# g8a9/multi-modal-emotion

Hardware: AMD Instinct MI355X
Metric: utterances/sec fwd+bwd (+clip_grad_norm_+AdamW inside the timed step), TAV (BERT+Wav2Vec2+VideoMAE) b=32, 1/2/4/8 MI355X (higher is better)
Workload: dtype bf16; 1 GPU; tav_nn.py TAV preset B (bert 12 L + wav2vec2 12 L / 768 + videomae 12 L / 768 on 16 frames + fusion 12 L), global batch 32 = 32 per GPU x 1, text 128 tok, audio 80000 samples, video 16x3x224x224 (104 fusion / 1464 encoder tokens), 547.0 GFLOP forward per utterance; global_batch=32, per_gpu_batch=32, parallelism=dp1, weights=random init (seeded), no checkpoints offline, launch=hipGraph replay

## Files before the change

### include/tavhip.h

```cpp
#ifndef TAVHIP_H
#define TAVHIP_H
#include <stdint.h>

#ifdef __cplusplus
extern "C" {
#endif

enum { TAV_F32 = 0, TAV_BF16 = 1, TAV_FP8 = 2  };
enum {
    TAV_ERR_NULL = -1,
    TAV_ERR_SHAPE = -2,
    TAV_ERR_DTYPE = -3,
    TAV_ERR_ALIGN = -4,
    TAV_ERR_NO_RCCL = -5
};

int tav_version(void);
const char* tav_error_string(int code);

typedef struct tav_gemm_nt_args {
    const void* A; const void* B; void* C;
    void* C_pre;
    const float* bias;
    const void* gelu_in;
// ... 120 lines not shown
int tav_embed_add_fwd(const float* x, const int64_t* ids, const float* table, float* out, int64_t rows, int64_t W, int64_t ntable,
                      void* stream);
int tav_embed_add_bwd(const float* dy, const int64_t* ids, float* dtable, float* partials, int64_t rows, int64_t W, int64_t ntable,
                      int32_t accumulate, void* stream);
int tav_embed_add_bwd_parts(int64_t rows);

typedef struct tav_text_embed_args {
    const int64_t* ids;
    const float* word; const float* pos; const float* type;
    const float* gamma; const float* beta;
    float* pre;
    int64_t* pos_ids;
    float* y_f32; void* y_lp; int32_t lp_dtype;
    float* mean; float* rstd;
    int64_t B, S, W, vocab, max_pos;
    int32_t pad_id;
    float eps;
} tav_text_embed_args;
int tav_text_embed_fwd(const tav_text_embed_args* args, void* stream);
int tav_scatter_add_rows(const float* d, const int64_t* idx, float* dtable, int64_t rows, int64_t W, int64_t ntable, void* stream);

int tav_patchify(const float* video, const int32_t* keep_idx, void* patches, int32_t dtype, int64_t B, int64_t F, int64_t H, int64_t W,
                 int64_t nkeep, void* stream);
int tav_mask_to_index(const uint8_t* mask, int32_t keep_value, int32_t* keep_idx, int32_t* counts, int64_t B, int64_t n, int64_t nkeep,
                      void* stream);
enum { TAV_RAGGED_OVER_TRUE = 1, TAV_RAGGED_OVER_KEEP = 2 };
int tav_ragged_lens(const uint8_t* mask, int32_t* true_cnt, int32_t* vid_lens, int32_t* av_lens, int32_t* status, int64_t B, int64_t ntok,
                    int64_t cap_true, int64_t cap_keep, int64_t base, void* stream);
int tav_gather_rows(const float* table, const int32_t* idx, float* out, int64_t rows, int64_t W, int64_t ntable, void* stream);

int tav_mean_pool_fwd(const float* x, float* y, int64_t B, int64_t S, int64_t W, void* stream);
int tav_mean_pool_bwd(const float* dy, float* dx, void* dx_lp, int32_t lp_dtype, int64_t B, int64_t S, int64_t W, void* stream);
int tav_mean_pool_fwd_len(const float* x, float* y, const int32_t* seq_lens, int64_t B, int64_t S, int64_t W, void* stream);
int tav_mean_pool_bwd_len(const float* dy, float* dx, void* dx_lp, int32_t lp_dtype, const int32_t* seq_lens, int64_t B, int64_t S, int64_t W,
                          void* stream);

int tav_head_fwd(const float* x, const float* W, const float* b, float* y, int64_t B, int64_t K, int64_t N, void* stream);
int tav_head_bwd(const float* x, const float* W, const float* dy, float* dx, float* dW, float* db, int64_t B, int64_t K, int64_t N,
                 int32_t accumulate, void* stream);
int tav_tanh_fwd(const float* x, float* y, int64_t n, void* stream);
int tav_tanh_bwd(const float* y, const float* dy, float* dx, int64_t n, void* stream);

int tav_cross_entropy(const float* logits, const int64_t* target, const float* class_weight , float* loss, float* dlogits,
                      int64_t B, int64_t C, float grad_scale, void* stream);

int tav_dropout_fwd(const float* x, float* y, uint8_t* mask, int64_t n, float p, uint64_t seed, uint64_t offset, void* stream);
int tav_dropout_fwd_dev(const float* x, float* y, uint8_t* mask, int64_t n, float p, const uint64_t* seed_state, uint64_t offset, void* stream);
int tav_dropout_bwd(const float* dy, const uint8_t* mask, float* dx, int64_t n, float p, void* stream);

#define TAV_SPECAUG_TAG_TIME 0x5350010000000000ull
#define TAV_SPECAUG_TAG_FEATURE 0x5350030000000000ull
int tav_specaug_draw(const uint8_t* valid, uint8_t* mask, int32_t* nspans, int64_t B, int64_t L, float prob, int64_t length, int64_t min_masks,
                     uint64_t seed, uint64_t tag, void* stream);
int tav_specaug_draw_dev(const uint8_t* valid, uint8_t* mask, int32_t* nspans, int64_t B, int64_t L, float prob, int64_t length,
                         int64_t min_masks, const uint64_t* seed_state, uint64_t tag, void* stream);
int tav_specaug_fwd(const float* x, const uint8_t* tmask, const uint8_t* fmask, const float* embed, float* y, int64_t B, int64_t T, int64_t H,
                    void* stream);
int64_t tav_specaug_bwd_ws_bytes(int64_t rows, int64_t H);
int tav_specaug_bwd(const float* dy, const uint8_t* tmask, const uint8_t* fmask, float* dx, float* dembed, void* workspace,
                    int64_t workspace_bytes, int64_t B, int64_t T, int64_t H, void* stream);

int tav_conv0_fwd(const float* wave, const float* w, const float* bias, void* y, int32_t y_dtype, int64_t B, int64_t T_in, int64_t T_out,
                  int64_t C, int64_t K, int64_t stride, void* stream);
int tav_conv0_bwd_w(const float* wave, const void* dy, int32_t dy_dtype, float* dw, float* dbias, float* partials, int64_t B, int64_t T_in,
                    int64_t T_out, int64_t C, int64_t K, int64_t stride, int32_t accumulate, void* stream);
int tav_conv0_bwd_partials(int64_t B, int64_t T_out, int64_t C, int64_t K);
int tav_gn_workspace_floats(int64_t B, int64_t C);
int tav_gn_gelu_fwd(const void* x, void* y, int32_t dtype, const float* gamma, const float* beta, float* stats, float* workspace, int64_t B,
                    int64_t T, int64_t C, float eps, void* stream);
int tav_gn_gelu_bwd(const void* x, const void* dy, void* dx, int32_t dtype, const float* gamma, const float* beta, const float* stats,
                    float* workspace, float* dgamma, float* dbeta, int64_t B, int64_t T, int64_t C, int32_t accumulate, void* stream);
int tav_gelu_fwd(const void* x, void* y, int32_t dtype, int64_t n, void* stream);
int tav_gelu_bwd(const void* x, const void* dy, void* dx, int32_t dtype, int64_t n, void* stream);
int tav_col2im_1d(const void* dcol, void* dx, const void* pre_act, int32_t dtype, int64_t B, int64_t T_in, int64_t T_out, int64_t C,
                  int64_t K, int64_t stride, void* stream);
int tav_group_pad(const void* x, int32_t x_dtype, void* xg, int32_t xg_dtype, int64_t B, int64_t T, int64_t H, int64_t G, int64_t pad_l,
                  int64_t pad_r, void* stream);
int tav_weight_norm_partials(int64_t H, int64_t Cg);
int tav_weight_norm_fwd(const float* v, const float* g, float* norms, float* partials, void* w, void* w_flip, int32_t dtype, int64_t H,
                        int64_t Cg, int64_t K, void* stream);
int tav_weight_norm_bwd(const float* v, const float* g, const float* norms, const float* dw_gemm, float* workspace, float* dv, float* dg,
                        int64_t H, int64_t Cg, int64_t K, int32_t accumulate, void* stream);

int tav_sumsq_partials(int32_t ntensors);
int tav_sumsq_multi(const float* const* ptrs, const int64_t* sizes, int32_t ntensors, float* partials, float* out_sumsq, void* stream);
int tav_clip_coef(const float* sumsq, float max_norm, float* coef_out, float* norm_out, void* stream);
int tav_adamw_multi(float* const* params, const float* const* grads, float* const* exp_avg, float* const* exp_avg_sq, const int64_t* sizes,
                    int32_t ntensors, const float* clip_coef , const float* lr, float beta1, float beta2, float eps, float weight_decay,
                    int32_t* step, float* bias_corr, void* stream);
int tav_optim_chunk_elems(void);
int tav_sumsq_chunked(const float* const* ptrs, const int64_t* sizes, const int32_t* chunk_prefix, int32_t ntensors, int32_t nchunks,
                      float* partials, float* out_sumsq, void* stream);
int tav_sum_partials(const float* partials, int64_t n, float* out, void* stream);
int tav_adamw_chunked(float* const* params, const float* const* grads, float* const* exp_avg, float* const* exp_avg_sq, const int64_t* sizes,
                      const int32_t* chunk_prefix, int32_t ntensors, int32_t nchunks, const float* clip_coef, const float* lr, float beta1,
                      float beta2, float eps, float weight_decay, int32_t* step, float* bias_corr, void* stream);

int tav_comm_rccl_version(int32_t* version);
int tav_comm_unique_id(void* out128);
int tav_comm_init_rank(void** comm, int32_t nranks, const void* unique_id128, int32_t rank);
int tav_comm_destroy(void* comm);
int tav_allreduce_bucket(void* buf, int64_t nbytes, int32_t dtype, void* comm, void* stream);

#ifdef __cplusplus
}
#endif
#endif
```

### multi-modal-emotion_amd/_lib.py

```python
import ctypes as C
import os

import torch

_HERE = os.path.dirname(os.path.abspath(__file__))
LIB_PATH = os.environ.get("TAV_LIB") or os.path.join(_HERE, "libtavhip.so")

TAV_F32, TAV_BF16, TAV_FP8 = 0, 1, 2
ABI_VERSION = 7

i32, i64, f32, vp = C.c_int32, C.c_int64, C.c_float, C.c_void_p


class GemmNTArgs(C.Structure):
    _fields_ = [("A", vp), ("B", vp), ("C", vp), ("C_pre", vp), ("bias", vp), ("gelu_in", vp), ("resid", vp),
                ("M", i64), ("N", i64), ("K", i64),
                ("lda", i64), ("ldb", i64), ("ldc", i64), ("ld_pre", i64), ("ld_gelu_in", i64), ("ld_resid", i64),
                ("nzb", i32), ("nzg", i32),
                ("a_zb", i64), ("a_zg", i64), ("b_zb", i64), ("b_zg", i64), ("c_zb", i64), ("c_zg", i64), ("bias_zg", i64),
                ("in_dtype", i32), ("out_dtype", i32), ("act", i32), ("accumulate", i32), ("alpha", f32),
                ("a_dequant", vp), ("b_dequant", vp), ("gelu_zb", i64), ("tile_m_hint", i32)]


class GemmTNArgs(C.Structure):
    _fields_ = [("A", vp), ("B", vp), ("slabs", vp), ("out", vp), ("dbias", vp), ("bias_partials", vp),
                ("N1", i64), ("N2", i64), ("lda", i64), ("ldb", i64), ("rows_per_batch", i64), ("nbatch", i64),
                ("a_zb", i64), ("b_zb", i64), ("chunk_rows", i32), ("nsplit", i32), ("perm_inner", i32), ("perm_outer", i32),
                ("dtype", i32), ("accumulate", i32), ("scale", f32)]


class GemmTNProblem(C.Structure):
    _fields_ = [("A", vp), ("B", vp), ("out", vp), ("dbias", vp), ("N1", i64), ("N2", i64), ("lda", i64), ("ldb", i64)]


class AttnArgs(C.Structure):
    _fields_ = [("q", vp), ("k", vp), ("v", vp), ("o", vp), ("key_mask", vp), ("lse", vp), ("corr", vp), ("o_soft", vp),
                ("dout", vp), ("dq", vp), ("dk", vp), ("dv", vp), ("delta", vp),
                ("B", i64), ("S", i64), ("nheads", i64),
                ("ld_q", i64), ("ld_k", i64), ("ld_v", i64), ("ld_o", i64), ("ld_do", i64), ("ld_dq", i64), ("ld_dk", i64), ("ld_dv", i64),
                ("dtype", i32), ("mask_mode", i32), ("scale", f32), ("q_prescaled", i32)]


class LnArgs(C.Structure):
    _fields_ = [("x", vp), ("x_dtype", i32), ("gamma", vp), ("beta", vp), ("y_f32", vp), ("y_lp", vp), ("lp_dtype", i32),
                ("mean", vp), ("rstd", vp),
                ("dy", vp), ("dy_dtype", i32), ("dx_add", vp), ("dx_f32", vp), ("dx_lp", vp),
                ("dgamma", vp), ("dbeta", vp), ("partials", vp), ("accumulate_params", i32),
                ("rows", i64), ("W", i64), ("ld_x", i64), ("ld_y", i64), ("ld_dy", i64), ("ld_dx", i64), ("eps", f32), ("act", i32),
                ("defer_param_reduce", i32)]


class LnReduceItem(C.Structure):
    _fields_ = [("partials", vp), ("dgamma", vp), ("dbeta", vp), ("nblocks", i32), ("W", i32), ("accumulate", i32), ("pad_", i32)]


LN_REDUCE_MAX = 64


class TextEmbedArgs(C.Structure):
    _fields_ = [("ids", vp), ("word", vp), ("pos", vp), ("type", vp), ("gamma", vp), ("beta", vp), ("pre", vp), ("pos_ids", vp),
                ("y_f32", vp), ("y_lp", vp), ("lp_dtype", i32), ("mean", vp), ("rstd", vp),
                ("B", i64), ("S", i64), ("W", i64), ("vocab", i64), ("max_pos", i64), ("pad_id", i32), ("eps", f32)]


_SIGS = {
    "tav_version": (C.c_int, []),
    "tav_error_string": (C.c_char_p, [C.c_int]),
    "tav_gemm_nt": (C.c_int, [C.POINTER(GemmNTArgs), vp]),
    "tav_gemm_nt_schedule": (C.c_int, [C.POINTER(GemmNTArgs), C.POINTER(i32), C.POINTER(i32), C.POINTER(i32)]),
    "tav_gemm_tn_splits": (C.c_int, [i64, i64, i64, i64, C.POINTER(i32), C.POINTER(i32)]),
    "tav_gemm_tn": (C.c_int, [C.POINTER(GemmTNArgs), vp]),
    "tav_gemm_tn_grouped": (C.c_int, [C.POINTER(GemmTNProblem), i32, i64, i32, vp]),
    "tav_gemm_tn_grouped_ws_bytes": (C.c_int64, [C.POINTER(GemmTNProblem), i32, i64, i32, i32]),
    "tav_gemm_tn_grouped_ws": (C.c_int, [C.POINTER(GemmTNProblem), i32, i64, i32, vp, i64, i32, vp]),
    "tav_colsum": (C.c_int, [vp, i32, i64, i64, i64, vp, i32, vp, i32, vp]),
    "tav_fp8_amax_partials": (C.c_int, [i64, i64]),
    "tav_fp8_amax": (C.c_int, [vp, i32, i64, i64, i64, vp, vp, vp]),
    "tav_fp8_quantize": (C.c_int, [vp, i32, i64, i64, i64, vp, vp, i64, vp, i64, i64, vp]),
    "tav_fp8_quantize_delayed": (C.c_int, [vp, i32, i64, i64, i64, vp, vp, i64, vp, i64, i64, vp]),
    "tav_fp8_roll_states": (C.c_int, [vp, i64, vp]),
    "tav_splitk_reduce": (C.c_int, [vp, vp, i32, i64, i32, vp]),
    "tav_comm_rccl_version": (C.c_int, [C.POINTER(i32)]),
    "tav_comm_unique_id": (C.c_int, [vp]),
    "tav_comm_init_rank": (C.c_int, [C.POINTER(vp), i32, vp, i32]),
    "tav_comm_destroy": (C.c_int, [vp]),
    "tav_allreduce_bucket": (C.c_int, [vp, i64, i32, vp, vp]),
    "tav_attn_fwd": (C.c_int, [C.POINTER(AttnArgs), vp]),
    "tav_attn_bwd": (C.c_int, [C.POINTER(AttnArgs), vp]),
    "tav_attn_fwd_len": (C.c_int, [C.POINTER(AttnArgs), vp, vp]),
    "tav_attn_bwd_len": (C.c_int, [C.POINTER(AttnArgs), vp, vp]),
    "tav_attn_probs": (C.c_int, [C.POINTER(AttnArgs), vp, vp, i64, vp]),
    "tav_head_scale": (C.c_int, [vp, vp, vp, i32, vp, i64, f32, i64, i64, i64, i64, i64, i64, vp]),
    "tav_ln_fwd": (C.c_int, [C.POINTER(LnArgs), vp]),
    "tav_ln_bwd": (C.c_int, [C.POINTER(LnArgs), vp]),
    "tav_ln_bwd_partials": (C.c_int, [i64]),
    "tav_ln_param_reduce_multi": (C.c_int, [C.POINTER(LnReduceItem), i32, vp]),
    "tav_cast_weight": (C.c_int, [vp, i64, i64, vp, i64, vp, i64, i32, vp]),
    "tav_cast_weights_multi": (C.c_int, [vp, i32, i32, vp]),
    "tav_cast_conv_weight": (C.c_int, [vp, i64, i64, i64, vp, vp, vp, i64, i32, vp]),
    "tav_zero_pad_rows": (C.c_int, [vp, i32, i64, i64, i64, i64, vp]),
    "tav_cast2d": (C.c_int, [vp, i32, i64, vp, i32, i64, i64, i64, vp]),
    "tav_transpose2d": (C.c_int, [vp, vp, i32, i64, i64, i64, vp]),
    "tav_add_f32": (C.c_int, [vp, vp, vp, vp, i32, i64, vp]),
    "tav_fill_f32": (C.c_int, [vp, f32, i64, vp]),
    "tav_embed_add_fwd": (C.c_int, [vp, vp, vp, vp, i64, i64, i64, vp]),
    "tav_embed_add_bwd": (C.c_int, [vp, vp, vp, vp, i64, i64, i64, i32, vp]),
    "tav_embed_add_bwd_parts": (C.c_int, [i64]),
    "tav_text_embed_fwd": (C.c_int, [C.POINTER(TextEmbedArgs), vp]),
    "tav_scatter_add_rows": (C.c_int, [vp, vp, vp, i64, i64, i64, vp]),
    "tav_gather_rows": (C.c_int, [vp, vp, vp, i64, i64, i64, vp]),
    "tav_patchify": (C.c_int, [vp, vp, vp, i32, i64, i64, i64, i64, i64, vp]),
    "tav_mask_to_index": (C.c_int, [vp, i32, vp, vp, i64, i64, i64, vp]),
    "tav_ragged_lens": (C.c_int, [vp, vp, vp, vp, vp, i64, i64, i64, i64, i64, vp]),
    "tav_mean_pool_fwd": (C.c_int, [vp, vp, i64, i64, i64, vp]),
    "tav_mean_pool_bwd": (C.c_int, [vp, vp, vp, i32, i64, i64, i64, vp]),
    "tav_mean_pool_fwd_len": (C.c_int, [vp, vp, vp, i64, i64, i64, vp]),
    "tav_mean_pool_bwd_len": (C.c_int, [vp, vp, vp, i32, vp, i64, i64, i64, vp]),
    "tav_head_fwd": (C.c_int, [vp, vp, vp, vp, i64, i64, i64, vp]),
    "tav_head_bwd": (C.c_int, [vp, vp, vp, vp, vp, vp, i64, i64, i64, i32, vp]),
    "tav_tanh_fwd": (C.c_int, [vp, vp, i64, vp]),
    "tav_tanh_bwd": (C.c_int, [vp, vp, vp, i64, vp]),
    "tav_cross_entropy": (C.c_int, [vp, vp, vp, vp, vp, i64, i64, f32, vp]),
    "tav_dropout_fwd": (C.c_int, [vp, vp, vp, i64, f32, C.c_uint64, C.c_uint64, vp]),
    "tav_dropout_fwd_dev": (C.c_int, [vp, vp, vp, i64, f32, vp, C.c_uint64, vp]),
    "tav_dropout_bwd": (C.c_int, [vp, vp, vp, i64, f32, vp]),
    "tav_specaug_draw": (C.c_int, [vp, vp, vp, i64, i64, f32, i64, i64, C.c_uint64, C.c_uint64, vp]),
    "tav_specaug_draw_dev": (C.c_int, [vp, vp, vp, i64, i64, f32, i64, i64, vp, C.c_uint64, vp]),
    "tav_specaug_fwd": (C.c_int, [vp, vp, vp, vp, vp, i64, i64, i64, vp]),
    "tav_specaug_bwd_ws_bytes": (C.c_int64, [i64, i64]),
    "tav_specaug_bwd": (C.c_int, [vp, vp, vp, vp, vp, vp, i64, i64, i64, i64, vp]),
    "tav_conv0_fwd": (C.c_int, [vp, vp, vp, vp, i32, i64, i64, i64, i64, i64, i64, vp]),
    "tav_conv0_bwd_w": (C.c_int, [vp, vp, i32, vp, vp, vp, i64, i64, i64, i64, i64, i64, i32, vp]),
    "tav_conv0_bwd_partials": (C.c_int, [i64, i64, i64, i64]),
    "tav_gn_workspace_floats": (C.c_int, [i64, i64]),
    "tav_gn_gelu_fwd": (C.c_int, [vp, vp, i32, vp, vp, vp, vp, i64, i64, i64, f32, vp]),
    "tav_gn_gelu_bwd": (C.c_int, [vp, vp, vp, i32, vp, vp, vp, vp, vp, vp, i64, i64, i64, i32, vp]),
    "tav_gelu_fwd": (C.c_int, [vp, vp, i32, i64, vp]),
    "tav_gelu_bwd": (C.c_int, [vp, vp, vp, i32, i64, vp]),
    "tav_col2im_1d": (C.c_int, [vp, vp, vp, i32, i64, i64, i64, i64, i64, i64, vp]),
    "tav_group_pad": (C.c_int, [vp, i32, vp, i32, i64, i64, i64, i64, i64, i64, vp]),
    "tav_weight_norm_partials": (C.c_int, [i64, i64]),
    "tav_weight_norm_fwd": (C.c_int, [vp, vp, vp, vp, vp, vp, i32, i64, i64, i64, vp]),
    "tav_weight_norm_bwd": (C.c_int, [vp, vp, vp, vp, vp, vp, vp, i64, i64, i64, i32, vp]),
    "tav_sumsq_partials": (C.c_int, [i32]),
    "tav_sumsq_multi": (C.c_int, [vp, vp, i32, vp, vp, vp]),
    "tav_clip_coef": (C.c_int, [vp, f32, vp, vp, vp]),
    "tav_adamw_multi": (C.c_int, [vp, vp, vp, vp, vp, i32, vp, vp, f32, f32, f32, f32, vp, vp, vp]),
    "tav_optim_chunk_elems": (C.c_int, []),
    "tav_sumsq_chunked": (C.c_int, [vp, vp, vp, i32, i32, vp, vp, vp]),
    "tav_sum_partials": (C.c_int, [vp, i64, vp, vp]),
    "tav_adamw_chunked": (C.c_int, [vp, vp, vp, vp, vp, vp, i32, i32, vp, vp, f32, f32, f32, f32, vp, vp, vp]),
}

_lib = None


def lib():
# ... 44 lines not shown
```

### multi-modal-emotion_amd/engine.py

```python
import os
import weakref

import torch

from . import ops

_EPOCH = [0]


def bump_weight_epoch():
    _EPOCH[0] += 1


class Policy:
    def __init__(self, name="bf16"):
        name = {"bfloat16": "bf16", "float32": "fp32", "f32": "fp32", "float8": "fp8", "e4m3": "fp8"}.get(name, name)
        if name not in ("bf16", "fp32", "fp8", "fp8-all", "fp8-wgrad8"):
            raise ValueError(f"unknown precision policy {name!r}")
        self.name = name
        self.lp = torch.float32 if name == "fp32" else torch.bfloat16
        self.f32 = name == "fp32"
        self.fp8 = name.startswith("fp8")
        self.fp8_stacks = () if not self.fp8 else (("video", "text", "audio", "fusion") if name == "fp8-all" else ("video",))
        self.fp8_wgrad8 = name in ("fp8-wgrad8", "fp8-all")
# ... 592 lines not shown
        ctx.ectx, ctx.geom, ctx.has_b = ectx, (B, T_in, Ci, Co, k, stride, T_out), b is not None
        ctx.chained = u_in is not None
        ctx.set_materialize_grads(False)
        ctx.save_for_backward(x, w, pre, u_in)
        return y, pre

    @staticmethod
    def backward(ctx, g, g_pre):
        x, w, pre, u_in = ctx.saved_tensors
        B, T_in, Ci, Co, k, stride, T_out = ctx.geom
        du = g_pre
        if g is not None:
            d2 = ops.gelu_bwd(pre, _c(g)) if pre is not None else _c(g)
            du = d2 if du is None else _c(du) + d2
        if du is None:
            return None, None, None, None, None, None, None
        _, w_t, w_ph = ctx.ectx.cache.conv(w, stride)
        P = CONV_PAD
        TP = T_out + 2 * P
        du_pad = _CONV_PADDED.pop(du.data_ptr(), None) if g is None else None
        if du_pad is not None and (tuple(du.shape) != (B, T_out, Co) or tuple(du.stride()) != (TP * Co, Co, 1) or tuple(du_pad.shape) != (B, TP, Co)):
            du_pad = None
        want_dx = ctx.needs_input_grad[1] if ctx.chained else ctx.needs_input_grad[0]
        phase = (CONV_PHASE_DGRAD[0] and w_ph is not None and want_dx and (k + stride - 1) // stride - 1 <= P
                 and (T_in - 1) // stride + 1 <= T_out + P)
        if du_pad is None:
            du = _c(du)
            if phase and du.numel() <= (1 << 23):
                du_pad = ops.zero_pad_rows(torch.empty(B, TP, Co, dtype=du.dtype, device=du.device), B, T_out, Co, P)
                du_pad[:, P:P + T_out].copy_(du)
            else:
                phase = False
        du_v = du_pad[:, P:P + T_out] if du_pad is not None else du
        za = TP * Co if du_pad is not None else T_out * Co
        dw = db = dx = dui = None
        if ctx.needs_input_grad[2]:
            dw = ops.gemm_tn(du_v, x, N1=Co, N2=k * Ci, lda=Co, ldb=stride * Ci, rows_per_batch=T_out, nbatch=B, a_zb=za, b_zb=T_in * Ci,
                             perm_inner=Ci, perm_outer=k, out_shape=(Co, Ci, k))
        if ctx.has_b and ctx.needs_input_grad[3]:
            db = ops.colsum(du_pad.view(B * TP, Co) if du_pad is not None else du.view(B * T_out, Co))
        if want_dx and phase:
            if ctx.chained:
                out = ops.zero_pad_rows(torch.empty(B, T_in + 2 * P, Ci, dtype=du_v.dtype, device=du_v.device), B, T_in, Ci, P)
                zc, obase = (T_in + 2 * P) * Ci, P * Ci
            else:
                out = torch.empty(B, T_in, Ci, dtype=du_v.dtype, device=du_v.device)
                zc, obase = T_in * Ci, 0
            oflat, aflat, uflat = out.view(-1), du_pad.view(-1), (u_in.reshape(-1) if ctx.chained else None)
            off = 0
            for r in range(stride):
                Q = (k - r + stride - 1) // stride
                Mr = (T_in - r + stride - 1) // stride
                ops.gemm_nt(aflat[(P - (Q - 1)) * Co:], w_ph[off:off + Ci * Q * Co], out=oflat[obase + r * Ci:], M=Mr, N=Ci, K=Q * Co, lda=Co, ldb=Q * Co,
                            ldc=stride * Ci, nzb=B, a_zb=TP * Co, c_zb=zc, gelu_in=uflat[r * Ci:] if ctx.chained else None,
                            ld_gelu=stride * Ci, gelu_zb=T_in * Ci)
                off += Ci * Q * Co
            if ctx.chained:
                dui = out[:, P:P + T_in]
                _CONV_PADDED[dui.data_ptr()] = out
            else:
                dx = out
        elif want_dx:
            dcol = ops.gemm_nt(_c(du_v).view(B * T_out, Co), w_t, out_shape=(B * T_out, k * Ci))
            d = ops.col2im_1d(dcol, B, T_in, T_out, Ci, k, stride, pre_act=u_in if ctx.chained else None)
            if ctx.chained:
                dui = d
            else:
                dx = d
        return dx, dui, dw, db, None, None, None


class PosConvFn(torch.autograd.Function):

    @staticmethod
    def forward(ctx, x, v, g, bias, B, T, G, ectx):
        pol = ectx.pol
        x = _c(x)
        H = x.shape[1]
        Cg, K = H // G, v.shape[2]
        w, _, norms = ectx.cache.posconv(v, g)
        pad = K // 2
        xg = ops.group_pad(x, B, T, H, G, pad, pad, pol.lp)
        TP = T + 2 * pad
        y, pre = ops.gemm_nt(xg, w, bias=bias, act=1, resid=x, want_pre=True, out_dtype=torch.float32, M=T, N=Cg, K=K * Cg, lda=Cg, ldb=K * Cg,
                             ldc=H, nzb=B, nzg=G, a_zb=G * TP * Cg, a_zg=TP * Cg, b_zg=Cg * K * Cg, c_zb=T * H, c_zg=Cg, bias_zg=Cg,
                             out_shape=(B * T, H))
        ctx.ectx, ctx.geom = ectx, (B, T, H, G, Cg, K)
        ctx.save_for_backward(xg, pre, v, g, norms)
        return y

    @staticmethod
    def backward(ctx, gout):
        xg, pre, v, g, norms = ctx.saved_tensors
        pol = ctx.ectx.pol
        B, T, H, G, Cg, K = ctx.geom
        gout = _c(gout)
        _, wf, _ = ctx.ectx.cache.posconv(v, g)
        du = ops.gelu_bwd(pre, gout)
        pad = K // 2
        dug = ops.group_pad(du, B, T, H, G, pad - 1, pad, pol.lp)
        TPd, TP = T + 2 * pad - 1, T + 2 * pad
        dx = ops.gemm_nt(dug, wf, resid=gout, out_dtype=torch.float32, M=T, N=Cg, K=K * Cg, lda=Cg, ldb=K * Cg, ldc=H, nzb=B, nzg=G,
                         a_zb=G * TPd * Cg, a_zg=TPd * Cg, b_zg=Cg * K * Cg, c_zb=T * H, c_zg=Cg, out_shape=(B * T, H))
        du_lp = _to_lp(pol, du)
        dw = torch.empty(G, Cg, K * Cg, dtype=torch.float32, device=du.device)
        for gi in range(G):
            ops.gemm_tn(du_lp[:, gi * Cg:], xg[:, gi], out=dw[gi], N1=Cg, N2=K * Cg, lda=H, ldb=Cg, rows_per_batch=T, nbatch=B, a_zb=T * H,
                        b_zb=G * TP * Cg)
        dv, dg = ops.weight_norm_bwd(v, g, norms, dw)
        dbias = ops.colsum(du)
        return dx, dv, dg.view_as(g), dbias, None, None, None, None


class ConcatSeqFn(torch.autograd.Function):

    @staticmethod
    def forward(ctx, B, *parts):
        W = parts[0].shape[-1]
        lens = [p.numel() // (B * W) for p in parts]
        Sf = sum(lens)
        out = torch.empty(B, Sf, W, dtype=torch.float32, device=parts[0].device)
        flat = out.view(B, Sf * W)
        off = 0
        for p, L in zip(parts, lens):
            ops.cast2d(_c(p).view(B, L * W), torch.float32, out=flat[:, off * W:(off + L) * W])
            off += L
        ctx.lens, ctx.W, ctx.B = lens, W, B
        return out

    @staticmethod
    def backward(ctx, g):
        B, W = ctx.B, ctx.W
        flat = _c(g).view(B, -1)
        outs, off = [], 0
        for L in ctx.lens:
            outs.append(ops.cast2d(flat[:, off * W:(off + L) * W], torch.float32).view(B * L, W))
            off += L
        return (None, *outs)


class TailFn(torch.autograd.Function):

    @staticmethod
    def forward(ctx, av_seq, t_pooled, aud_seq, vid_seq, B, S_av, S_aud, S_vid, p_drop, seed, rand_w, rand_b, bert_w, bert_b, aud_w, aud_b,
                vid_w, vid_b, lin_w, lin_b, av_lens=None, vid_lens=None):
        W = 768
        pooled = [ops.mean_pool_fwd(_c(av_seq), B, S_av, seq_lens=av_lens), _c(t_pooled), ops.mean_pool_fwd(_c(aud_seq), B, S_aud),
                  ops.mean_pool_fwd(_c(vid_seq), B, S_vid, seq_lens=vid_lens)]
        norms = [(rand_w, rand_b), (bert_w, bert_b), (aud_w, aud_b), (vid_w, vid_b)]
        cat = torch.empty(B, 4 * W, dtype=torch.float32, device=av_seq.device)
        stats = []
        for j, (x, (w, b)) in enumerate(zip(pooled, norms)):
            y32, _, mean, rstd = ops.ln_fwd(x, w.detach(), b.detach(), 1e-5, want_f32=True)
            ops.cast2d(y32, torch.float32, out=cat[:, j * W:(j + 1) * W])
            stats += [mean, rstd]
        mask = None
        feat = cat
        if p_drop > 0.0:
            feat, mask = ops.dropout_fwd(cat, p_drop, seed, 0)
        logits = ops.head_fwd(feat, lin_w.detach(), lin_b.detach())
        ctx.geom = (B, S_av, S_aud, S_vid, p_drop)
        ctx.lens = (av_lens, vid_lens)
        ctx.save_for_backward(feat, mask, lin_w, *pooled, *stats, rand_w, rand_b, bert_w, bert_b, aud_w, aud_b, vid_w, vid_b)
        return logits

    @staticmethod
    def backward(ctx, g):
        B, S_av, S_aud, S_vid, p_drop = ctx.geom
        sv = ctx.saved_tensors
        feat, mask, lin_w = sv[:3]
        pooled, stats, nw = sv[3:7], sv[7:15], sv[15:23]
        W = 768
        dfeat, dW, db = ops.head_bwd(feat, lin_w, _c(g))
        if mask is not None:
            dfeat = ops.dropout_bwd(dfeat, mask, p_drop)
        dpool, dparams = [], []
        for j in range(4):
            dy = ops.cast2d(dfeat[:, j * W:(j + 1) * W], torch.float32)
            dx, _, dg, dbt = ops.ln_bwd(dy, pooled[j], nw[2 * j], nw[2 * j + 1], stats[2 * j], stats[2 * j + 1], want_f32=True)
            dpool.append(dx)
            dparams += [dg, dbt]
        av_lens, vid_lens = ctx.lens
        d_av, _ = ops.mean_pool_bwd(dpool[0], B, S_av, seq_lens=av_lens)
        d_aud, _ = ops.mean_pool_bwd(dpool[2], B, S_aud)
        d_vid, _ = ops.mean_pool_bwd(dpool[3], B, S_vid, seq_lens=vid_lens)
        return (d_av, dpool[1], d_aud, d_vid, None, None, None, None, None, None, *dparams, dW, db, None, None)


class HeadFn(torch.autograd.Function):

    @staticmethod
# ... 154 lines not shown
```

### multi-modal-emotion_amd/ops.py

```python
import ctypes as C
import os

import torch

from . import _lib as L
from ._lib import check, dt, lib, ptr, stream

_ws = {}


def workspace(name, nfloats, device):
    key = (name, torch.cuda.current_stream().cuda_stream, str(device))
    t = _ws.get(key)
    if t is None or t.numel() < nfloats:
        t = torch.empty(max(int(nfloats), 1), dtype=torch.float32, device=device)
        _ws[key] = t
    return t


def clear_workspaces():
    _ws.clear()


_prof = None
# ... 657 lines not shown
        check(lib().tav_specaug_draw_dev(ptr(valid), ptr(mask), ptr(nspans), B, L, prob, length, min_masks, ptr(seed), tag, stream()), "specaug_draw_dev")
    else:
        check(lib().tav_specaug_draw(ptr(valid), ptr(mask), ptr(nspans), B, L, prob, length, min_masks, seed, tag, stream()), "specaug_draw")
    return (mask, nspans) if want_nspans else mask


def specaug_fwd(x, tmask, fmask, embed, B, T):
    H = x.shape[-1]
    tmask, fmask = _mask_bytes(tmask, (B, T), "specaug_fwd"), _mask_bytes(fmask, (B, H), "specaug_fwd")
    y = torch.empty_like(x)
    check(lib().tav_specaug_fwd(ptr(x), ptr(tmask), ptr(fmask), ptr(embed), ptr(y), B, T, H, stream()), "specaug_fwd")
    return y


def specaug_bwd(dy, tmask, fmask, B, T, want_dembed=True):
    H = dy.shape[-1]
    tmask, fmask = _mask_bytes(tmask, (B, T), "specaug_bwd"), _mask_bytes(fmask, (B, H), "specaug_bwd")
    dx = torch.empty_like(dy)
    dembed = part = None
    nbytes = 0
    if want_dembed:
        dembed = torch.empty(H, dtype=torch.float32, device=dy.device)
        nbytes = lib().tav_specaug_bwd_ws_bytes(B * T, H)
        part = workspace("specaug_part", nbytes // 4, dy.device)
    check(lib().tav_specaug_bwd(ptr(dy), ptr(tmask), ptr(fmask), ptr(dx), ptr(dembed), ptr(part), nbytes, B, T, H, stream()), "specaug_bwd")
    return dx, dembed


def conv0_fwd(wave, w, bias, T_out, stride, dtype):
    B, T_in = wave.shape
    Cc, K = w.shape[0], w.shape[-1]
    y = torch.empty(B, T_out, Cc, dtype=dtype, device=wave.device)
    check(lib().tav_conv0_fwd(ptr(wave), ptr(w), ptr(bias), ptr(y), dt(dtype), B, T_in, T_out, Cc, K, stride, stream()), "conv0_fwd")
    return y


def conv0_bwd_w(wave, dy, K, stride, want_bias):
    B, T_in = wave.shape
    _, T_out, Cc = dy.shape
    part = workspace("conv0_part", lib().tav_conv0_bwd_partials(B, T_out, Cc, K), wave.device)
    dw = torch.empty(Cc, 1, K, dtype=torch.float32, device=wave.device)
    db = torch.empty(Cc, dtype=torch.float32, device=wave.device) if want_bias else None
    check(lib().tav_conv0_bwd_w(ptr(wave), ptr(dy), dt(dy), ptr(dw), ptr(db), ptr(part), B, T_in, T_out, Cc, K, stride, 0, stream()), "conv0_bwd_w")
    return dw, db


def gn_gelu_fwd(x, gamma, beta, eps):
    B, T, Cc = x.shape
    y = torch.empty_like(x)
    stats = torch.empty(B, Cc, 2, dtype=torch.float32, device=x.device)
    wsb = workspace("gn_ws", lib().tav_gn_workspace_floats(B, Cc), x.device)
    check(lib().tav_gn_gelu_fwd(ptr(x), ptr(y), dt(x), ptr(gamma), ptr(beta), ptr(stats), ptr(wsb), B, T, Cc, eps, stream()), "gn_gelu_fwd")
    return y, stats


def gn_gelu_bwd(x, dy, gamma, beta, stats):
    B, T, Cc = x.shape
    dx = torch.empty_like(x)
    dg = torch.empty(Cc, dtype=torch.float32, device=x.device)
    db = torch.empty(Cc, dtype=torch.float32, device=x.device)
    wsb = workspace("gn_ws", lib().tav_gn_workspace_floats(B, Cc), x.device)
    check(lib().tav_gn_gelu_bwd(ptr(x), ptr(dy), ptr(dx), dt(x), ptr(gamma), ptr(beta), ptr(stats), ptr(wsb), ptr(dg), ptr(db), B, T, Cc, 0, stream()), "gn_gelu_bwd")
    return dx, dg, db


def gelu_bwd(x, dy):
    dx = torch.empty_like(x)
    check(lib().tav_gelu_bwd(ptr(x), ptr(dy), ptr(dx), dt(x), x.numel(), stream()), "gelu_bwd")
    return dx


def col2im_1d(dcol, B, T_in, T_out, Cc, K, stride, pre_act=None):
    dx = torch.empty(B, T_in, Cc, dtype=dcol.dtype, device=dcol.device)
    check(lib().tav_col2im_1d(ptr(dcol), ptr(dx), ptr(pre_act), dt(dcol), B, T_in, T_out, Cc, K, stride, stream()), "col2im_1d")
    return dx


def group_pad(x, B, T, H, G, pad_l, pad_r, dtype):
    xg = torch.empty(B, G, pad_l + T + pad_r, H // G, dtype=dtype, device=x.device)
    check(lib().tav_group_pad(ptr(x), dt(x), ptr(xg), dt(dtype), B, T, H, G, pad_l, pad_r, stream()), "group_pad")
    return xg


def weight_norm_fwd(v, g, dtype):
    H, Cg, K = v.shape
    norms = torch.empty(K, dtype=torch.float32, device=v.device)
    part = workspace("wn_part", lib().tav_weight_norm_partials(H, Cg) * K, v.device)
    G = H // Cg
    w = torch.empty(G, Cg, K * Cg, dtype=dtype, device=v.device)
    wf = torch.empty(G, Cg, K * Cg, dtype=dtype, device=v.device)
    check(lib().tav_weight_norm_fwd(ptr(v), ptr(g), ptr(norms), ptr(part), ptr(w), ptr(wf), dt(dtype), H, Cg, K, stream()), "weight_norm_fwd")
    return w, wf, norms


def weight_norm_bwd(v, g, norms, dw_gemm):
    H, Cg, K = v.shape
    wsb = workspace("wn_bwd", H * Cg * K + lib().tav_weight_norm_partials(H, Cg) * K + K, v.device)
    dv = torch.empty_like(v)
    dg = torch.empty(K, dtype=torch.float32, device=v.device)
    check(lib().tav_weight_norm_bwd(ptr(v), ptr(g), ptr(norms), ptr(dw_gemm), ptr(wsb), ptr(dv), ptr(dg), H, Cg, K, 0, stream()), "weight_norm_bwd")
    return dv, dg
```

Before: 416.4 utterances/s.

## Add windowed grouped-conv kernels for Wav2Vec2 positional conv fwd, dgrad and wgrad

Adds dedicated HIP kernels for the Wav2Vec2 positional grouped convolution. Each block stages a sliding input window in LDS and reuses it across all K taps rather than running a generic strided GEMM. The bias, GELU and residual epilogue stays fused. The weight gradient becomes a single kernel over all groups that accumulates over batch and time tiles, replacing a per-group Python loop of gemm_tn launches. Unsupported shapes fall back to the old GEMM path, at the cost of extra kernel code and LDS-size constraints.

```diff
diff --git a/include/tavhip.h b/include/tavhip.h
--- a/include/tavhip.h
+++ b/include/tavhip.h
@@ -226,6 +226,21 @@
 int tav_weight_norm_bwd(const float* v, const float* g, const float* norms, const float* dw_gemm, float* workspace, float* dv, float* dg,
                         int64_t H, int64_t Cg, int64_t K, int32_t accumulate, void* stream);
 
+typedef struct tav_posconv_args {
+    const void* x; const void* w;
+    float* out;
+    float* pre;
+    const float* bias;
+    const float* resid;
+    int64_t B, T, TP, H, G, K;
+    int64_t ld_out;
+    int32_t dtype;
+    int32_t act;
+} tav_posconv_args;
+int tav_posconv_nt(const tav_posconv_args* args, void* stream);
+int tav_posconv_wgrad(const void* du, int64_t ld_du, const void* xg, float* dw, int64_t B, int64_t T, int64_t TP, int64_t H, int64_t G,
+                      int64_t K, int32_t dtype, void* stream);
+
 int tav_sumsq_partials(int32_t ntensors);
 int tav_sumsq_multi(const float* const* ptrs, const int64_t* sizes, int32_t ntensors, float* partials, float* out_sumsq, void* stream);
 int tav_clip_coef(const float* sumsq, float max_norm, float* coef_out, float* norm_out, void* stream);
diff --git a/multi-modal-emotion_amd/_lib.py b/multi-modal-emotion_amd/_lib.py
--- a/multi-modal-emotion_amd/_lib.py
+++ b/multi-modal-emotion_amd/_lib.py
@@ -8,6 +8,7 @@
 
 TAV_F32, TAV_BF16, TAV_FP8 = 0, 1, 2
 ABI_VERSION = 7
+TAV_ERR_SHAPE = -2
 
 i32, i64, f32, vp = C.c_int32, C.c_int64, C.c_float, C.c_void_p
 
@@ -31,6 +32,11 @@
 
 class GemmTNProblem(C.Structure):
     _fields_ = [("A", vp), ("B", vp), ("out", vp), ("dbias", vp), ("N1", i64), ("N2", i64), ("lda", i64), ("ldb", i64)]
+
+
+class PosConvArgs(C.Structure):
+    _fields_ = [("x", vp), ("w", vp), ("out", vp), ("pre", vp), ("bias", vp), ("resid", vp),
+                ("B", i64), ("T", i64), ("TP", i64), ("H", i64), ("G", i64), ("K", i64), ("ld_out", i64), ("dtype", i32), ("act", i32)]
 
 
 class AttnArgs(C.Structure):
@@ -73,6 +79,8 @@
     "tav_gemm_tn_grouped": (C.c_int, [C.POINTER(GemmTNProblem), i32, i64, i32, vp]),
     "tav_gemm_tn_grouped_ws_bytes": (C.c_int64, [C.POINTER(GemmTNProblem), i32, i64, i32, i32]),
     "tav_gemm_tn_grouped_ws": (C.c_int, [C.POINTER(GemmTNProblem), i32, i64, i32, vp, i64, i32, vp]),
+    "tav_posconv_nt": (C.c_int, [C.POINTER(PosConvArgs), vp]),
+    "tav_posconv_wgrad": (C.c_int, [vp, i64, vp, vp, i64, i64, i64, i64, i64, i64, i32, vp]),
     "tav_colsum": (C.c_int, [vp, i32, i64, i64, i64, vp, i32, vp, i32, vp]),
     "tav_fp8_amax_partials": (C.c_int, [i64, i64]),
     "tav_fp8_amax": (C.c_int, [vp, i32, i64, i64, i64, vp, vp, vp]),
diff --git a/multi-modal-emotion_amd/csrc/posconv.hip b/multi-modal-emotion_amd/csrc/posconv.hip
--- /dev/null
+++ b/multi-modal-emotion_amd/csrc/posconv.hip
@@ -0,0 +1,395 @@
+#include "common.h"
+#include <type_traits>
+#include "tavhip_internal.h"
+
+namespace tav {
+
+struct PosConvNT {
+    const char* X; const char* W; float* C; float* Cpre; const float* bias; const float* resid;
+    int B, T, TP, G, K;
+    long ldc;
+    int gelu;
+    float alpha;
+    int row_tiles, bblocks, win_bytes;
+};
+
+TAV_DEV int pc_swz(int row, int chunk) { return chunk ^ ((row >> 1) & 7); }
+
+template <int TN, int EW>
+__global__ __launch_bounds__(256, 1) void posconv_nt_kernel(const PosConvNT p) {
+    constexpr int CG = 16 * TN, CPR = CG / 8, BM = 128, TM = 4, NB = 2 * EW, NST = 4, RING = 64 * 128;
+    constexpr int PW = TN > 2 ? 2 : 1;
+    extern __shared__ __attribute__((aligned(16))) char smem[];
+    const int tid = threadIdx.x, lane = tid & 63, wave = tid >> 6;
+    const int g = lane >> 4, i = lane & 15;
+    const int wm = wave & 1, we = wave >> 1;
+
+    const int id = xcd_remap(blockIdx.x, gridDim.x);
+    const int per = p.row_tiles * p.bblocks;
+    const int zg = to_sgpr(id / per);
+    const int rem = id - zg * per;
+    const int bb = to_sgpr(rem / p.row_tiles);
+    const int rt = rem - bb * p.row_tiles;
+    const int m0 = rt * BM, b0 = bb * NB;
+    char* const sWin = smem;
+    char* const sRing = smem + NB * p.win_bytes;
+
+    const long ldb_bytes = (long)p.K * CG * 2;
+    const char* const Wb = p.W + (long)zg * CG * ldb_bytes;
+    const int lr = lane >> 3, lc = lane & 7;
+    unsigned gb[PW];
+#pragma unroll
+    for (int j = 0; j < PW; ++j) {
+        const int r = (wave + 4 * j) * 8 + lr;
+        const int rs = r < CG ? r : CG - 1;
+        gb[j] = (unsigned)(rs * ldb_bytes + pc_swz(r, lc) * 16);
+    }
+    const unsigned ldsR = __builtin_amdgcn_readfirstlane(lds_addr(sRing) + wave * 1024);
+    auto stage_w = [&](int j, unsigned ko, int buf) { glds16_m0(Wb + ko, gb[j], ldsR + buf * RING + j * 4096); };
+    const int nk = p.K * CG / 64;
+#pragma unroll
+    for (int t = 0; t < NST - 1; ++t)
+        if (t < nk) {
+#pragma unroll
+            for (int j = 0; j < PW; ++j) stage_w(j, (unsigned)t * 128u, t);
+        }
+
+    const int nch = (BM + p.K - 1) * CPR;
+    auto win_off = [&](int c) -> int {
+        if constexpr (CG == 64) { const int row = c >> 3; return row * 128 + (pc_swz(row, c & 7) << 4); }
+        else return c * 16;
+    };
+#pragma unroll 1
+    for (int e = 0; e < NB; ++e) {
+        const int b = b0 + e;
+        const char* src = p.X + (((long)b * p.G + zg) * p.TP + m0) * (CG * 2);
+        char* dst = sWin + e * p.win_bytes;
+#pragma unroll 1
+        for (int c0 = 0; c0 < nch; c0 += 256 * 8) {
+            uint4 v[8];
+#pragma unroll
+            for (int j = 0; j < 8; ++j) {
+                const int c = c0 + j * 256 + tid;
+                v[j] = make_uint4(0, 0, 0, 0);
+                if (c < nch && b < p.B && m0 + c / CPR < p.TP) v[j] = *reinterpret_cast<const uint4*>(src + (long)c * 16);
+            }
+#pragma unroll
+            for (int j = 0; j < 8; ++j) {
+                const int c = c0 + j * 256 + tid;
+                if (c < nch) *reinterpret_cast<uint4*>(dst + win_off(c)) = v[j];
+            }
+        }
+    }
+
+    f32x4 acc[EW][TN][TM];
+#pragma unroll
+    for (int e = 0; e < EW; ++e)
+#pragma unroll
+        for (int a = 0; a < TN; ++a)
+#pragma unroll
+            for (int b = 0; b < TM; ++b) acc[e][a][b] = f32x4{0.f, 0.f, 0.f, 0.f};
+
+    int off_b[2][TN];
+#pragma unroll
+    for (int s2 = 0; s2 < 2; ++s2)
+#pragma unroll
+        for (int t = 0; t < TN; ++t) { const int r = t * 16 + i; off_b[s2][t] = r * 128 + pc_swz(r, 4 * s2 + g) * 16; }
+    int arow[EW][TM];
+#pragma unroll
+    for (int e = 0; e < EW; ++e)
+#pragma unroll
+        for (int t = 0; t < TM; ++t) {
+            const int row = wm * 64 + t * 16 + i;
+            arow[e][t] = (we * EW + e) * p.win_bytes + (CG == 64 ? row * 128 : (row * CG + 8 * g) * 2);
+        }
+    auto a_frag = [&](int e, int t, int kt, int s2) -> uint4 {
+        if constexpr (CG == 64) {
+            const int row = wm * 64 + t * 16 + i + kt;
+            return *reinterpret_cast<const uint4*>(sWin + arow[e][t] + kt * 128 + (pc_swz(row, 4 * s2 + g) << 4));
+        } else {
+            return *reinterpret_cast<const uint4*>(sWin + arow[e][t] + kt * 128 + s2 * 64);
+        }
+    };
+
+    uint4 fa0[EW][TM], fa1[EW][TM], fb0[TN], fb1[TN];
+    auto ktile = [&](int kt, int cur, auto prefetch) {
+        if constexpr (decltype(prefetch)::value) asm volatile("s_waitcnt vmcnt(%0)" ::"n"((NST - 2) * PW) : "memory");
+        else wait_vmcnt0();
+        __syncthreads();
+        const char* cB = sRing + cur * RING;
+        const unsigned ko = (unsigned)(kt + NST - 1) * 128u;
+        const int nxt = (cur + NST - 1) % NST;
+#pragma unroll
+        for (int t = 0; t < TN; ++t) fb0[t] = *reinterpret_cast<const uint4*>(cB + off_b[0][t]);
+#pragma unroll
+        for (int e = 0; e < EW; ++e)
+#pragma unroll
+            for (int t = 0; t < TM; ++t) fa0[e][t] = a_frag(e, t, kt, 0);
+#pragma unroll
+        for (int t = 0; t < TN; ++t) fb1[t] = *reinterpret_cast<const uint4*>(cB + off_b[1][t]);
+#pragma unroll
+        for (int e = 0; e < EW; ++e)
+#pragma unroll
+            for (int t = 0; t < TM; ++t) fa1[e][t] = a_frag(e, t, kt, 1);
+        __builtin_amdgcn_sched_barrier(0);
+#pragma unroll
+        for (int tn = 0; tn < TN; ++tn) {
+#pragma unroll
+            for (int e = 0; e < EW; ++e)
+#pragma unroll
+                for (int tm = 0; tm < TM; ++tm) mma16<bf16>(fb0[tn], fa0[e][tm], acc[e][tn][tm]);
+            if constexpr (decltype(prefetch)::value) {
+                if (tn < PW) {
+                    __builtin_amdgcn_sched_barrier(0);
+                    stage_w(tn, ko, nxt);
+                    __builtin_amdgcn_sched_barrier(0);
+                }
+            }
+        }
+#pragma unroll
+        for (int tn = 0; tn < TN; ++tn)
+#pragma unroll
+            for (int e = 0; e < EW; ++e)
+#pragma unroll
+                for (int tm = 0; tm < TM; ++tm) mma16<bf16>(fb1[tn], fa1[e][tm], acc[e][tn][tm]);
+    };
+    static_assert(PW <= TN, "one DMA piece per MFMA group");
+    int cur = 0, kt = 0;
+    for (; kt + NST - 1 < nk; ++kt) { ktile(kt, cur, std::true_type{}); cur = cur + 1 == NST ? 0 : cur + 1; }
+    for (; kt < nk; ++kt) { ktile(kt, cur, std::false_type{}); cur = cur + 1 == NST ? 0 : cur + 1; }
+
+    const float alpha = p.alpha;
+#pragma unroll
+    for (int e = 0; e < EW; ++e) {
+        const int b = b0 + we * EW + e;
+        if (b >= p.B) continue;
+#pragma unroll
+        for (int tn = 0; tn < TN; ++tn) {
+            const int n = tn * 16 + 4 * g;
+            f32x4 bv = {0.f, 0.f, 0.f, 0.f};
+            if (p.bias) bv = ld4(p.bias + zg * CG + n);
+#pragma unroll
+            for (int tm = 0; tm < TM; ++tm) {
+                const int m = m0 + wm * 64 + tm * 16 + i;
+                if (m >= p.T) continue;
+                const long o = ((long)b * p.T + m) * p.ldc + zg * CG + n;
+                f32x4 v = acc[e][tn][tm];
+                v = v * alpha + bv;
+                if (p.Cpre) st4(p.Cpre + o, v);
+                if (p.gelu) { v[0] = gelu_t<bf16>(v[0]); v[1] = gelu_t<bf16>(v[1]); v[2] = gelu_t<bf16>(v[2]); v[3] = gelu_t<bf16>(v[3]); }
+                if (p.resid) v += ld4(p.resid + o);
+                st4(p.C + o, v);
+            }
+        }
+    }
+}
+
+struct PosConvWG {
+    const char* DU; const char* X; float* DW;
+    int B, T, TP, G, K;
+    long ld_du;
+    int nblk;
+};
+
+template <int CG> TAV_DEV int img_off(int row, int col) {
+    if constexpr (CG == 64) {
+        const int r2 = row + (col >> 6), c = (col & 63) >> 3;
+        return r2 * 128 + ((c ^ (((r2 >> 1) & 3) << 1)) << 4) + (col & 7) * 2;
+    } else {
+        return (row * CG + col) * 2;
+    }
+}
+template <int CG> TAV_DEV uint4 img_frag(const char* img, int krow0, int col0, int lane) {
+    const int g = lane >> 4, i = lane & 15, q = i >> 2, pp = i & 3;
+    const int r0 = krow0 + 4 * g + q, col = col0 + 4 * pp;
+    const uint2 lo = lds_read_tr16(img + img_off<CG>(r0, col));
+    const uint2 hi = lds_read_tr16(img + img_off<CG>(r0 + 16, col));
+    return make_uint4(lo.x, lo.y, hi.x, hi.y);
+}
+
+template <int TN1, int NT2>
+__global__ __launch_bounds__(256, 1) void posconv_wgrad_kernel(const PosConvWG p) {
+    constexpr int CG = 16 * TN1, CPR = CG / 8, NKK = 64 * NT2, NTAP = NKK / CG, TT = 256, XR = TT + NTAP - 1;
+    static_assert(NKK % CG == 0, "a column block is a whole number of taps");
+    constexpr int NDU = TT * CPR, NCH = NDU + XR * CPR, NLD = (NCH + 255) / 256;
+    constexpr int DU_BYTES = TT * CG * 2, BUF = DU_BYTES + XR * CG * 2;
+    extern __shared__ __attribute__((aligned(16))) char smem[];
+    const int tid = threadIdx.x, lane = tid & 63, wave = tid >> 6;
+    const int g = lane >> 4, i = lane & 15;
+    const int id = xcd_remap(blockIdx.x, gridDim.x);
+    const int zg = id / p.nblk, blk = id - zg * p.nblk;
+    const int tap0 = blk * NTAP;
+    const int ntt = (p.T + TT - 1) / TT, nstages = p.B * ntt;
+
+    auto gload = [&](int s, uint4* v) {
+        const int b = s / ntt, tt0 = (s - b * ntt) * TT;
+        const char* du = p.DU + (((long)b * p.T + tt0) * p.ld_du + zg * CG) * 2;
+        const char* x = p.X + (((long)b * p.G + zg) * p.TP + tap0 + tt0) * (CG * 2);
+#pragma unroll
+        for (int j = 0; j < NLD; ++j) {
+            const int c = j * 256 + tid;
+            v[j] = make_uint4(0, 0, 0, 0);
+            if (c < NDU) {
+                const int row = c / CPR, cc = c - row * CPR;
+                if (tt0 + row < p.T) v[j] = *reinterpret_cast<const uint4*>(du + (long)row * p.ld_du * 2 + cc * 16);
+            } else if (c < NCH) {
+                const int c2 = c - NDU;
+                if (tap0 + tt0 + c2 / CPR < p.TP) v[j] = *reinterpret_cast<const uint4*>(x + (long)c2 * 16);
+            }
+        }
+    };
+    auto lstore = [&](int buf, const uint4* v) {
+        char* base = smem + buf * BUF;
+#pragma unroll
+        for (int j = 0; j < NLD; ++j) {
+            const int c = j * 256 + tid;
+            if (c < NDU) {
+                const int row = c / CPR, cc = c - row * CPR;
+                *reinterpret_cast<uint4*>(base + img_off<CG>(row, cc * 8)) = v[j];
+            } else if (c < NCH) {
+                const int c2 = c - NDU, row = c2 / CPR, cc = c2 - row * CPR;
+                *reinterpret_cast<uint4*>(base + DU_BYTES + img_off<CG>(row, cc * 8)) = v[j];
+            }
+        }
+    };
+
+    f32x4 acc[TN1][NT2], tot[TN1][NT2];
+#pragma unroll
+    for (int a = 0; a < TN1; ++a)
+#pragma unroll
+        for (int b = 0; b < NT2; ++b) { acc[a][b] = f32x4{0.f, 0.f, 0.f, 0.f}; tot[a][b] = f32x4{0.f, 0.f, 0.f, 0.f}; }
+
+    uint4 v[NLD];
+    gload(0, v);
+    lstore(0, v);
+    __syncthreads();
+    const int col_w = wave * 16 * NT2;
+    for (int s = 0; s < nstages; ++s) {
+        const bool more = s + 1 < nstages;
+        if (more) gload(s + 1, v);
+        __builtin_amdgcn_sched_barrier(0);
+        const int tl = s % ntt;
+        int rows = p.T - tl * TT; rows = rows < TT ? rows : TT;
+        const int nsteps = (rows + 31) / 32;
+        const char* duimg = smem + (s & 1) * BUF;
+        const char* ximg = duimg + DU_BYTES;
+        uint4 f1[TN1], f2[NT2], n1[TN1], n2[NT2];
+#pragma unroll
+        for (int a = 0; a < TN1; ++a) f1[a] = img_frag<CG>(duimg, 0, a * 16, lane);
+#pragma unroll
+        for (int b = 0; b < NT2; ++b) f2[b] = img_frag<CG>(ximg, 0, col_w + b * 16, lane);
+        for (int st = 0; st < nsteps; ++st) {
+            const int tn0 = st + 1 < nsteps ? (st + 1) * 32 : st * 32;
+#pragma unroll
+            for (int a = 0; a < TN1; ++a) n1[a] = img_frag<CG>(duimg, tn0, a * 16, lane);
+#pragma unroll
+            for (int b = 0; b < NT2; ++b) n2[b] = img_frag<CG>(ximg, tn0, col_w + b * 16, lane);
+#pragma unroll
+            for (int a = 0; a < TN1; ++a)
+#pragma unroll
+                for (int b = 0; b < NT2; ++b) mma16<bf16>(f2[b], f1[a], acc[a][b]);
+#pragma unroll
+            for (int a = 0; a < TN1; ++a) f1[a] = n1[a];
+#pragma unroll
+            for (int b = 0; b < NT2; ++b) f2[b] = n2[b];
+        }
+        if (tl == ntt - 1) {
+#pragma unroll
+            for (int a = 0; a < TN1; ++a)
+#pragma unroll
+                for (int b = 0; b < NT2; ++b) { tot[a][b] += acc[a][b]; acc[a][b] = f32x4{0.f, 0.f, 0.f, 0.f}; }
+        }
+        if (more) lstore((s + 1) & 1, v);
+        __syncthreads();
+    }
+
+    const long n2_total = (long)p.K * CG;
+#pragma unroll
+    for (int a = 0; a < TN1; ++a) {
+        const long row = (long)zg * CG + a * 16 + i;
+#pragma unroll
+        for (int b = 0; b < NT2; ++b) st4(p.DW + row * n2_total + (long)blk * NKK + col_w + b * 16 + 4 * g, tot[a][b]);
+    }
+}
+
+static constexpr long PC_LDS_MAX = 160 * 1024;
+
+}
+
+using namespace tav;
+
+static int posconv_geometry(int64_t B, int64_t T, int64_t TP, int64_t H, int64_t G, int64_t K, int32_t dtype, int* cg) {
+    if (B <= 0 || T <= 0 || TP <= 0 || H <= 0 || G <= 0 || K <= 0) return TAV_ERR_SHAPE;
+    if (dtype != TAV_BF16 && dtype != TAV_F32) return TAV_ERR_DTYPE;
+    if (dtype != TAV_BF16) return TAV_ERR_SHAPE;
+    if (H % G) return TAV_ERR_SHAPE;
+    const int64_t Cg = H / G;
+    if (Cg % 16 || Cg > 64) return TAV_ERR_SHAPE;
+    if (TP < T + K - 1) return TAV_ERR_SHAPE;
+    if ((K * Cg) % 64) return TAV_ERR_SHAPE;
+    if (B > (1 << 20) || T > (1 << 24) || K > 4096 || G > 4096) return TAV_ERR_SHAPE;
+    *cg = (int)Cg;
+    return 0;
+}
+
+extern "C" int tav_posconv_nt(const tav_posconv_args* a, void* stream_) {
+    hipStream_t stream = (hipStream_t)stream_;
+    if (!a || !a->x || !a->w || !a->out) return TAV_ERR_NULL;
+    int Cg = 0;
+    const int e = posconv_geometry(a->B, a->T, a->TP, a->H, a->G, a->K, a->dtype, &Cg);
+    if (e) return e;
+    if (a->ld_out < a->H) return TAV_ERR_SHAPE;
+    if (a->ld_out % 4) return TAV_ERR_ALIGN;
+    if (a->act != 0 && a->act != 1) return TAV_ERR_SHAPE;
+    const long win = (128 + a->K - 1) * (long)Cg * 2;
+    const long ring = 4 * 64 * 128;
+    int ew = (a->B > 2 && 4 * win + ring <= PC_LDS_MAX) ? 2 : 1;
+    if (2 * ew * win + ring > PC_LDS_MAX) return TAV_ERR_SHAPE;
+    PosConvNT p;
+    p.X = (const char*)a->x; p.W = (const char*)a->w; p.C = a->out; p.Cpre = a->pre; p.bias = a->bias; p.resid = a->resid;
+    p.B = (int)a->B; p.T = (int)a->T; p.TP = (int)a->TP; p.G = (int)a->G; p.K = (int)a->K;
+    p.ldc = a->ld_out; p.gelu = a->act & 1; p.alpha = 1.f;
+    p.row_tiles = (int)((a->T + 127) / 128); p.bblocks = (int)((a->B + 2 * ew - 1) / (2 * ew)); p.win_bytes = (int)win;
+    const dim3 grid((unsigned)((long)a->G * p.row_tiles * p.bblocks)), block(256);
+    const size_t lds = (size_t)(2 * ew * win + ring);
+#define TAV_PC_NT(TN_)                                                                                              \
+    do {                                                                                                            \
+        if (ew == 2) hipLaunchKernelGGL((posconv_nt_kernel<TN_, 2>), grid, block, lds, stream, p);                  \
+        else hipLaunchKernelGGL((posconv_nt_kernel<TN_, 1>), grid, block, lds, stream, p);                          \
+    } while (0)
+    switch (Cg / 16) {
+        case 1: TAV_PC_NT(1); break;
+        case 2: TAV_PC_NT(2); break;
+        case 3: TAV_PC_NT(3); break;
+        default: TAV_PC_NT(4); break;
+    }
+#undef TAV_PC_NT
+    return (int)hipGetLastError();
+}
+
+extern "C" int tav_posconv_wgrad(const void* du, int64_t ld_du, const void* xg, float* dw, int64_t B, int64_t T, int64_t TP, int64_t H, int64_t G,
+                                 int64_t K, int32_t dtype, void* stream_) {
+    hipStream_t stream = (hipStream_t)stream_;
+    if (!du || !xg || !dw) return TAV_ERR_NULL;
+    int Cg = 0;
+    const int e = posconv_geometry(B, T, TP, H, G, K, dtype, &Cg);
+    if (e) return e;
+    if (ld_du < H) return TAV_ERR_SHAPE;
+    if (ld_du % 8) return TAV_ERR_ALIGN;
+    const int nt2 = Cg == 48 ? 6 : 4;
+    const int nkk = 64 * nt2, ntap = nkk / Cg;
+    if (K % ntap) return TAV_ERR_SHAPE;
+    PosConvWG p;
+    p.DU = (const char*)du; p.X = (const char*)xg; p.DW = dw;
+    p.B = (int)B; p.T = (int)T; p.TP = (int)TP; p.G = (int)G; p.K = (int)K; p.ld_du = ld_du;
+    p.nblk = (int)(K / ntap);
+    const dim3 grid((unsigned)((long)G * p.nblk)), block(256);
+    const size_t lds = (size_t)2 * (256 + 256 + ntap - 1) * Cg * 2;
+    switch (Cg / 16) {
+        case 1: hipLaunchKernelGGL((posconv_wgrad_kernel<1, 4>), grid, block, lds, stream, p); break;
+        case 2: hipLaunchKernelGGL((posconv_wgrad_kernel<2, 4>), grid, block, lds, stream, p); break;
+        case 3: hipLaunchKernelGGL((posconv_wgrad_kernel<3, 6>), grid, block, lds, stream, p); break;
+        default: hipLaunchKernelGGL((posconv_wgrad_kernel<4, 4>), grid, block, lds, stream, p); break;
+    }
+    return (int)hipGetLastError();
+}
diff --git a/multi-modal-emotion_amd/engine.py b/multi-modal-emotion_amd/engine.py
--- a/multi-modal-emotion_amd/engine.py
+++ b/multi-modal-emotion_amd/engine.py
@@ -698,9 +698,7 @@
         pad = K // 2
         xg = ops.group_pad(x, B, T, H, G, pad, pad, pol.lp)
         TP = T + 2 * pad
-        y, pre = ops.gemm_nt(xg, w, bias=bias, act=1, resid=x, want_pre=True, out_dtype=torch.float32, M=T, N=Cg, K=K * Cg, lda=Cg, ldb=K * Cg,
-                             ldc=H, nzb=B, nzg=G, a_zb=G * TP * Cg, a_zg=TP * Cg, b_zg=Cg * K * Cg, c_zb=T * H, c_zg=Cg, bias_zg=Cg,
-                             out_shape=(B * T, H))
+        y, pre = ops.posconv_nt(xg, w, B=B, T=T, H=H, G=G, K=K, bias=bias, resid=x, act=1, want_pre=True)
         ctx.ectx, ctx.geom = ectx, (B, T, H, G, Cg, K)
         ctx.save_for_backward(xg, pre, v, g, norms)
         return y
@@ -716,13 +714,9 @@
         pad = K // 2
         dug = ops.group_pad(du, B, T, H, G, pad - 1, pad, pol.lp)
         TPd, TP = T + 2 * pad - 1, T + 2 * pad
-        dx = ops.gemm_nt(dug, wf, resid=gout, out_dtype=torch.float32, M=T, N=Cg, K=K * Cg, lda=Cg, ldb=K * Cg, ldc=H, nzb=B, nzg=G,
-                         a_zb=G * TPd * Cg, a_zg=TPd * Cg, b_zg=Cg * K * Cg, c_zb=T * H, c_zg=Cg, out_shape=(B * T, H))
+        dx = ops.posconv_nt(dug, wf, B=B, T=T, H=H, G=G, K=K, resid=gout)
         du_lp = _to_lp(pol, du)
-        dw = torch.empty(G, Cg, K * Cg, dtype=torch.float32, device=du.device)
-        for gi in range(G):
-            ops.gemm_tn(du_lp[:, gi * Cg:], xg[:, gi], out=dw[gi], N1=Cg, N2=K * Cg, lda=H, ldb=Cg, rows_per_batch=T, nbatch=B, a_zb=T * H,
-                        b_zb=G * TP * Cg)
+        dw = ops.posconv_wgrad(du_lp, xg, B=B, T=T, H=H, G=G, K=K)
         dv, dg = ops.weight_norm_bwd(v, g, norms, dw)
         dbias = ops.colsum(du)
         return dx, dv, dg.view_as(g), dbias, None, None, None, None
diff --git a/multi-modal-emotion_amd/ops.py b/multi-modal-emotion_amd/ops.py
--- a/multi-modal-emotion_amd/ops.py
+++ b/multi-modal-emotion_amd/ops.py
@@ -763,6 +763,54 @@
     return xg
 
 
+def posconv_window_enabled():
+    return os.environ.get("TAV_POSCONV_WINDOW", "1") != "0"
+
+
+def _posconv_supported(xg, Cg):
+    return posconv_window_enabled() and xg.dtype == torch.bfloat16 and Cg % 16 == 0 and Cg <= 64
+
+
+def posconv_nt(xg, w, *, B, T, H, G, K, bias=None, resid=None, act=0, want_pre=False):
+    Cg, TP = H // G, xg.shape[2]
+    if _posconv_supported(xg, Cg):
+        out = torch.empty(B * T, H, dtype=torch.float32, device=xg.device)
+        pre = torch.empty_like(out) if want_pre else None
+        a = L.PosConvArgs()
+        a.x, a.w, a.out, a.pre, a.bias, a.resid = ptr(xg), ptr(w), ptr(out), ptr(pre), ptr(bias), ptr(resid)
+        a.B, a.T, a.TP, a.H, a.G, a.K, a.ld_out, a.dtype, a.act = B, T, TP, H, G, K, H, dt(xg), act
+        assert w.dtype == xg.dtype and (bias is None or bias.dtype == torch.float32) and (resid is None or resid.dtype == torch.float32)
+        rc = []
+        nz, M, N, KK = B * G, T, Cg, K * Cg
+        nbytes = nz * ((M * KK + N * KK) * 2 + M * N * (4 * (2 if want_pre else 1) + (4 if resid is not None else 0)))
+        _prof_launch("gemm_nt", "bf16", 2.0 * M * N * KK * nz, nbytes, lambda: rc.append(lib().tav_posconv_nt(C.byref(a), stream())))
+        if rc[0] == 0:
+            return (out, pre) if want_pre else out
+        if rc[0] != L.TAV_ERR_SHAPE:
+            check(rc[0], "posconv_nt")
+    return gemm_nt(xg, w, bias=bias, act=act, resid=resid, want_pre=want_pre, out_dtype=torch.float32, M=T, N=Cg, K=K * Cg, lda=Cg, ldb=K * Cg,
+                   ldc=H, nzb=B, nzg=G, a_zb=G * TP * Cg, a_zg=TP * Cg, b_zg=Cg * K * Cg, c_zb=T * H, c_zg=Cg, bias_zg=Cg if bias is not None else 0,
+                   out_shape=(B * T, H))
+
+
+def posconv_wgrad(du_lp, xg, *, B, T, H, G, K):
+    Cg, TP = H // G, xg.shape[2]
+    dw = torch.empty(G, Cg, K * Cg, dtype=torch.float32, device=du_lp.device)
+    if _posconv_supported(xg, Cg) and du_lp.dtype == xg.dtype:
+        rc = []
+        tokens = B * T
+        _prof_launch("gemm_tn", "bf16", 2.0 * tokens * Cg * K * Cg * G, G * (tokens * (Cg + K * Cg) * 2 + 4 * Cg * K * Cg),
+                     lambda: rc.append(lib().tav_posconv_wgrad(ptr(du_lp), du_lp.stride(0), ptr(xg), ptr(dw), B, T, TP, H, G, K, dt(xg), stream())))
+        if rc[0] == 0:
+            return dw
+        if rc[0] != L.TAV_ERR_SHAPE:
+            check(rc[0], "posconv_wgrad")
+    for gi in range(G):
+        gemm_tn(du_lp[:, gi * Cg:], xg[:, gi], out=dw[gi], N1=Cg, N2=K * Cg, lda=H, ldb=Cg, rows_per_batch=T, nbatch=B, a_zb=T * H,
+                b_zb=G * TP * Cg)
+    return dw
+
+
 def weight_norm_fwd(v, g, dtype):
     H, Cg, K = v.shape
     norms = torch.empty(K, dtype=torch.float32, device=v.device)
```

Result: no change. 420.3 utterances/s (median of 6 runs) (+0.9%).
